# multiview-stitcher/multiview-stitcher

Hardware: AMD Instinct MI355X
Metric: Mvoxels/s register+fuse, 3D tile grid (higher is better)
Workload: dtype u16 in/out, f32 accumulate, f64 coordinates

## Files before the change

### multiview-stitcher_amd/csrc/mvs_context.hip

```cpp
#include "mvs_internal.h"
#include <vector>
#include <algorithm>

#include <algorithm>
#include <cstring>

static MvsContext g_ctx[MVS_MAX_DEVICES * MVS_MAX_LANES];

MvsContext* mvs_ctx(int device) {
    if (device < 0 || (device & 0xff) >= MVS_MAX_DEVICES || (device >> 8) >= MVS_MAX_LANES) return nullptr;
    return &g_ctx[mvs_ctx_index(device)];
}

int mvs_fail(MvsContext* c, int code, const char* fmt, ...) {
    char buf[1024];
    va_list ap;
    va_start(ap, fmt);
    vsnprintf(buf, sizeof(buf), fmt, ap);
    va_end(ap);
    if (c) { c->last_error = buf; c->last_code = code; }
    return code;
}

int mvs_check_ready(int device, MvsContext** out) {
// ... 126 lines not shown
    if (hipEventRecord(c->pinned_ev[k], c->stream) == hipSuccess) c->pinned_pending[k] = true;
    else hipStreamSynchronize(c->stream);
}

static size_t pool_round(uint64_t nbytes) {
    if (nbytes == 0) nbytes = 1;
    const size_t q = nbytes >= ((size_t)1 << 20) ? ((size_t)2 << 20) : 4096;
    return (nbytes + q - 1) / q * q;
}

static void pool_flush(MvsContext* c) {
    if (c->pool_free.empty()) return;
    hipStreamSynchronize(c->stream);
    for (auto& kv : c->pool_free) hipFree(kv.second);
    c->pool_free.clear();
    c->pool_cached_bytes = 0;
}

struct MvsBoolOption { const char* key; bool MvsContext::* field; };
static const MvsBoolOption kBoolOptions[] = {
    {"force_generic", &MvsContext::force_generic},
    {"no_regions", &MvsContext::no_regions},
    {"deconv_general", &MvsContext::deconv_general},
    {"dct_general", &MvsContext::dct_general},
    {"rows_v1", &MvsContext::rows_v1},
    {"cb_mask_count", &MvsContext::cb_mask_count},
    {"cb_mask_closed_form", &MvsContext::cb_mask_closed_form},
    {"fuse_mixed", &MvsContext::fuse_mixed},
    {"serial_classes", &MvsContext::serial_classes},
    {"reg_unfused", &MvsContext::reg_unfused},
    {"ssim_two_pass", &MvsContext::ssim_two_pass},
    {"ssim_f32", &MvsContext::ssim_f32},
    {"ssim_prune", &MvsContext::ssim_prune},
    {"materialize_shifts", &MvsContext::materialize_shifts},
    {"cb_exact", &MvsContext::cb_exact},
    {"cb_blend_generic", &MvsContext::cb_blend_generic},
    {"cb_nosplit", &MvsContext::cb_nosplit},
    {"cb_unpaired", &MvsContext::cb_unpaired},
    {"fft_no_pair", &MvsContext::fft_no_pair},
    {"fft_no_slab", &MvsContext::fft_no_slab},
    {"fft_no_line", &MvsContext::fft_no_line},
};
static int set_option(MvsContext* c, const char* key, int64_t value) {
    for (const MvsBoolOption& e : kBoolOptions)
        if (!strcmp(key, e.key)) {
            c->*e.field = value != 0;
            return MVS_OK;
        }
    if (!strcmp(key, "pool_cache_limit_mb")) {
        std::lock_guard<std::mutex> plock(c->pool_mu);
        c->pool_cache_limit = (size_t)std::max<int64_t>(value, 0) << 20;
        if (c->pool_cached_bytes > c->pool_cache_limit) pool_flush(c);
        return MVS_OK;
    }
    if (!strcmp(key, "cb_taps_f64")) {
        if (value < 0 || value > 3) return mvs_fail(c, MVS_ERR_INVALID_ARG, "mvs_set_option: cb_taps_f64 is 0, 1, 2 or 3");
        c->cb_taps = (int)value;
        return MVS_OK;
    }
    if (!strcmp(key, "fft_slab_axes")) {
        if (value < 0 || value > 7) return mvs_fail(c, MVS_ERR_INVALID_ARG, "mvs_set_option: fft_slab_axes is a mask of 3 bits");
        c->fft_slab_axes = (int)value;
        return MVS_OK;
    }
    if (!strcmp(key, "psf_batch")) {
        if (value < 0) return mvs_fail(c, MVS_ERR_INVALID_ARG, "mvs_set_option: psf_batch is 0 (automatic) or a number of beads");
        c->psf_batch = value;
        return MVS_OK;
    }
    if (!strcmp(key, "feather_slab_planes")) {
        if (value < 0) return mvs_fail(c, MVS_ERR_INVALID_ARG, "mvs_set_option: feather_slab_planes is 0 (automatic) or a number of planes");
        c->feather_slab_planes = value;
        return MVS_OK;
    }
    if (!strcmp(key, "ablate")) {
        c->ablate = (int)value;
        return MVS_OK;
    }
    return mvs_fail(c, MVS_ERR_INVALID_ARG, "mvs_set_option: unknown key '%s'", key);
}
struct MvsCounter { const char* key; double MvsContext::* real; long long MvsContext::* count; };
static const MvsCounter kCounters[] = {
    {"reg_alg_bytes", &MvsContext::reg_alg_bytes, nullptr},
    {"reg_alg_bytes_full", &MvsContext::reg_alg_bytes_full, nullptr},
    {"reg_pairs", nullptr, &MvsContext::reg_pairs},
    {"reg_candidates", nullptr, &MvsContext::reg_candidates},
    {"reg_rewalks", nullptr, &MvsContext::reg_rewalks},
    {"reg_pruned", nullptr, &MvsContext::reg_pruned},
    {"reg_cand_volumes", &MvsContext::reg_cand_volumes, nullptr},
    {"reg_slab_pairs", nullptr, &MvsContext::reg_slab_pairs},
    {"reg_rank_hist", nullptr, &MvsContext::reg_rank_hist},
    {"reg_rank_sort16", nullptr, &MvsContext::reg_rank_sort16},
    {"reg_rank_sort32", nullptr, &MvsContext::reg_rank_sort32},
    {"cb_mask_views", nullptr, &MvsContext::cb_mask_views},
    {"cb_mask_boxes", nullptr, &MvsContext::cb_mask_boxes},
    {"cb_line_launches", nullptr, &MvsContext::cb_line_launches},
    {"cb_overflows_redone", nullptr, &MvsContext::cb_overflows},
    {"cb_exact_chunks", nullptr, &MvsContext::cb_exact_chunks},
    {"cb_exact_large_chunks", nullptr, &MvsContext::cb_exact_large_chunks},
    {"cb_exact_paired_launches", nullptr, &MvsContext::cb_exact_paired_launches},
    {"cb_exact_lds_launches", nullptr, &MvsContext::cb_exact_lds_launches},
    {"cb_exact_tap_launches", nullptr, &MvsContext::cb_exact_tap_launches},
    {"fuse_rows_chunks", nullptr, &MvsContext::fuse_rows_chunks},
    {"fuse_region_chunks", nullptr, &MvsContext::fuse_region_chunks},
    {"fuse_column_chunks", nullptr, &MvsContext::fuse_column_chunks},
    {"fuse_generic_chunks", nullptr, &MvsContext::fuse_generic_chunks},
    {"fuse_weighted_chunks", nullptr, &MvsContext::fuse_weighted_chunks},
};

extern "C" {

const char* mvs_version(void) { return "mvs_hip 0.1 (gfx950)"; }

int mvs_device_count(void) {
    int n = 0;
    if (hipGetDeviceCount(&n) != hipSuccess) return 0;
    return n;
}

int mvs_init(int device) {
    MvsContext* c = mvs_ctx(device);
// ... 21 lines not shown
            hipDeviceProp_t prop;
            MVS_HIP_TRY(c, hipGetDeviceProperties(&prop, mvs_hip_device(device)));
            const int ncu = prop.multiProcessorCount;
            const bool xcd = !strncmp(ev, "xcd", 3);
            const int k = std::max(1, std::min(8, atoi(ev + (xcd ? 3 : 6))));
            std::vector<uint32_t> mask((size_t)(ncu + 31) / 32, 0u);
            for (int i = 0; i < ncu; ++i) {
                bool on;
                if (xcd) { const int x = i % 8, first = (lane * k) % 8; on = ((x - first + 8) % 8) < k; }
                else { const int slot = (i / 8) % 8, first = (lane * k) % 8; on = ((slot - first + 8) % 8) < k; }
                if (on) mask[(size_t)i / 32] |= 1u << (i % 32);
            }
            if (hipExtStreamCreateWithCUMask(&c->own_stream, (uint32_t)mask.size(), mask.data()) == hipSuccess) masked = true;
            else (void)hipGetLastError();
        }
        if (!masked) MVS_HIP_TRY(c, hipStreamCreateWithFlags(&c->own_stream, hipStreamNonBlocking));
    }
    MVS_HIP_TRY(c, hipEventCreate(&c->ev_start));
    MVS_HIP_TRY(c, hipEventCreate(&c->ev_stop));
    MVS_HIP_TRY(c, hipEventCreateWithFlags(&c->pinned_ev[0], hipEventDisableTiming));
    MVS_HIP_TRY(c, hipEventCreateWithFlags(&c->pinned_ev[1], hipEventDisableTiming));
    c->pinned_pending[0] = c->pinned_pending[1] = false;
    c->stream = c->own_stream;
    c->device = device;
    c->pool_cache_limit = ((device >> 8) ? (size_t)4 : (size_t)32) << 30;
    if (((device >> 8) & 0xff) == 0) {
        size_t f = 0, t = 0;
        if (hipMemGetInfo(&f, &t) == hipSuccess) c->pool_cache_limit = std::max(c->pool_cache_limit, t / 2);
        else (void)hipGetLastError();
    }
    {
        static const char* const env_switch[][2] = {{"MVS_SSIM_PRUNE", "ssim_prune"},   {"MVS_SSIM_F32", "ssim_f32"},
                                                    {"MVS_FUSE_MIXED", "fuse_mixed"},   {"MVS_FFT_SLAB_AXES", "fft_slab_axes"},
                                                    {"MVS_FFT_NO_SLAB", "fft_no_slab"}, {"MVS_FFT_NO_PAIR", "fft_no_pair"}};
        for (const auto& e : env_switch) {
            const char* ev = getenv(e[0]);
            if (ev && *ev) (void)set_option(c, e[1], atoi(ev));
        }
    }
    c->ready = true;
    c->last_error.clear();
    c->last_code = 0;
    return MVS_OK;
}

#ifdef MVS_PROFILING_ABLATIONS
extern "C++" bool mvs_dup_kernel(const char* tag) {
    static const std::string list = [] { const char* e = getenv("MVS_DUP_KERNELS"); return std::string(",") + (e ? e : "") + ","; }();
    return list.find(std::string(",") + tag + ",") != std::string::npos;
}
#endif

void mvs_shutdown(int device) {
    MvsContext* c = mvs_ctx(device);
    if (!c || !c->ready) return;
    std::lock_guard<std::recursive_mutex> lock(c->mu);
    hipSetDevice(mvs_hip_device(device));
    hipStreamSynchronize(c->stream);
    if (((device >> 8) & 0xff) == 0) mvs_transfer_shutdown(mvs_hip_device(device));
    {
        std::lock_guard<std::mutex> plock(c->pool_mu);
        for (auto& kv : c->pool_free) hipFree(kv.second);
        c->pool_free.clear();
        c->pool_cached_bytes = 0;
        c->pool_live.clear();
    }
    for (auto& s : c->dev) {
// ... 376 lines not shown
```

### multiview-stitcher_amd/csrc/mvs_internal.h

```cpp
#pragma once
#include <hip/hip_runtime.h>

#include <cstdarg>
#include <cstdint>
#include <cstdio>
#include <map>
#include <mutex>
#include <unordered_map>
#include <string>
#include <vector>

#include "mvs_hip.h"

#define MVS_MAX_DEVICES 16
#define MVS_MAX_LANES 16
static inline int mvs_hip_device(int id) { return id & 0xff; }
static inline int mvs_ctx_index(int id) { return ((id >> 8) & 0xff) * MVS_MAX_DEVICES + (id & 0xff); }

struct MvsScratch {
    void* ptr = nullptr;
    size_t cap = 0;
};

struct MvsContext {
    int device = -1;
    bool ready = false;
    hipStream_t own_stream = nullptr;
    hipStream_t stream = nullptr;
    hipEvent_t ev_start = nullptr, ev_stop = nullptr;
    bool timing_valid = false;
    int ablate = 0;
    bool force_generic = false;
    double reg_alg_bytes = 0.0;
    double reg_alg_bytes_full = 0.0;
    long long reg_pairs = 0, reg_candidates = 0, reg_pruned = 0;
    long long reg_slab_pairs = 0;
    long long reg_rank_hist = 0, reg_rank_sort16 = 0, reg_rank_sort32 = 0;
    double reg_cand_volumes = 0.0;
    hipStream_t aux_stream[4] = {nullptr, nullptr, nullptr, nullptr};
    hipEvent_t ev_fork = nullptr, ev_join[4] = {nullptr, nullptr, nullptr, nullptr};
    bool fuse_mixed = false;
    bool serial_classes = false;
    bool reg_unfused = false;
    bool ssim_f32 = true;
    long long reg_rewalks = 0;
    bool ssim_prune = true;
    bool fft_no_pair = false;
    bool ssim_two_pass = false;
    bool materialize_shifts = false;
    std::recursive_mutex mu;
    std::string last_error;
    MvsScratch dev[16];
    void* pinned = nullptr;
    size_t pinned_cap = 0;
    void* pinned2 = nullptr;
    size_t pinned2_cap = 0;
    hipEvent_t pinned_ev[2] = {nullptr, nullptr};
    hipEvent_t ticket_ev[32] = {};
    uint32_t ticket_next = 0;
    bool pinned_pending[2] = {false, false};
    int last_code = 0;
    void* mbox_host = nullptr;
    void* mbox_dev = nullptr;
    size_t mbox_cap = 0;
    uint64_t mbox_gen = 0;
    bool cb_mask_closed_form = false;
    bool cb_mask_count = false;
    long long cb_mask_views = 0, cb_mask_boxes = 0;
    bool cb_exact = false;
    bool cb_blend_generic = false;
    int cb_taps = 1;
    int* cb_flag_host = nullptr;
    int* cb_flag_dev = nullptr;
    long long cb_overflows = 0, cb_line_launches = 0;
    long long cb_exact_chunks = 0, cb_exact_large_chunks = 0, cb_exact_paired_launches = 0, cb_exact_lds_launches = 0, cb_exact_tap_launches = 0;
    bool cb_nosplit = false;
    bool cb_unpaired = false;
    int fft_slab_axes = 4;
// ... 130 lines not shown
```

### multiview-stitcher_amd/csrc/mvs_prune_search.h

```cpp
#pragma once

#include <algorithm>
#include <cmath>

#if defined(__HIPCC__)
#define MVS_WALK_HD __host__ __device__
#else
#define MVS_WALK_HD
#endif

constexpr int kSelRot = 7;

struct WalkItem { int tx, ty, zs, z0, z1, y0, x0; };

template <int WIN>
struct WalkGeom {
    static constexpr int TY = 16, TX = 56, H = WIN / 2, PAD = (WIN - 1) / 2;
    static constexpr int kMinSeg = 8;
    int nz, ny, nx, zseg, cz, cy, cx, nty, ntx, nzs, nitems;

    MVS_WALK_HD static constexpr int crop(int n) { return n - 2 * PAD; }
    MVS_WALK_HD static constexpr int lesser(int a, int b) { return a < b ? a : b; }
    MVS_WALK_HD static constexpr int tiles(int ny, int nx) { return ((crop(ny) + TY - 1) / TY) * ((crop(nx) + TX - 1) / TX); }
    MVS_WALK_HD WalkGeom(int nz_, int ny_, int nx_, int zseg_)
        : nz(nz_), ny(ny_), nx(nx_), zseg(zseg_), cz(crop(nz_)), cy(crop(ny_)), cx(crop(nx_)), nty((cy + TY - 1) / TY), ntx((cx + TX - 1) / TX),
          nzs((cz + zseg_ - 1) / zseg_), nitems(nty * ntx * nzs) {}
    MVS_WALK_HD WalkItem item(int i) const {
        WalkItem w;
        w.tx = i % ntx; w.ty = (i / ntx) % nty; w.zs = i / (ntx * nty);
        w.z0 = PAD + w.zs * zseg;
        w.z1 = lesser(w.z0 + zseg, nz - PAD);
        w.y0 = PAD + w.ty * TY; w.x0 = PAD + w.tx * TX;
        return w;
    }
    MVS_WALK_HD static int group_first(int grp, int K) { return grp * K; }
    MVS_WALK_HD static int rotated(int res, int grp, int K) { return (res + kSelRot * grp) % K; }
    MVS_WALK_HD static int item_of(int grp, int res, int K) { return group_first(grp, K) + rotated(res, grp, K); }
    MVS_WALK_HD static int residue_of(int item, int K) { return (((item % K) - kSelRot * (item / K)) % K + K) % K; }
    MVS_WALK_HD double voxels(int i) const {
        const WalkItem w = item(i);
        return (double)(w.z1 - w.z0) * (double)lesser(TY, cy - w.ty * TY) * (double)lesser(TX, cx - w.tx * TX);
    }
    static int zseg_for(int nz, int ny, int nx, int budget, int sharers = 1) {
        const int cz = crop(nz);
        const int nzs = std::max(1, std::min(budget / std::max(tiles(ny, nx) * sharers, 1), (cz + kMinSeg - 1) / kMinSeg));
        return (cz + nzs - 1) / nzs;
    }
};

constexpr int kPruneMaxCand = 16;
constexpr double kPruneMarginF32 = 1e-3;

template <int WIN>
inline void prune_residue_volumes(const WalkGeom<WIN>& g, int K, double vol_res[32]) {
    for (int r = 0; r < 32; ++r) vol_res[r] = 0.0;
    for (int item = 0; item < g.nitems; ++item) vol_res[WalkGeom<WIN>::residue_of(item, K)] += g.voxels(item);
}

class PruneSearch {
public:
    PruneSearch(int n, const bool* takes_part, int K, const double vol_res[32], double Ntot, double slack, double margin, double im1_min)
        : nb(n), K(K), kAll(K == 32 ? 0xffffffffu : 0xffffu), Ntot(Ntot), slack(slack), margin(margin), im1_min(im1_min) {
        for (int r = 0; r < 32; ++r) this->vol_res[r] = vol_res[r];
        for (int j = 0; j < kPruneMaxCand; ++j) {
            in[j] = j < n && takes_part[j];
            acc[j] = 0.0; amx[j] = -INFINITY; ahn[j] = 0; done[j] = 0; masks[j] = 0; dropped[j] = false; again[j] = false; ub[j] = 0.0; racc[j] = 0.0;
        }
    }

    bool next_round(unsigned int out[kPruneMaxCand]) {
        bool more = false;
        if (phase == kFirst) {
            for (int j = 0; j < nb; ++j) { masks[j] = in[j] ? 0x0001u : 0u; more = more || in[j]; }
        } else if (phase == kRounds && round < 34) {
            more = plan();
        }
        if (!more && phase != kFirst && phase != kOver) {
            more = phase == kRounds && select_rewalk();
            phase = more ? kRewalk : kOver;
        }
        for (int j = 0; j < kPruneMaxCand; ++j) out[j] = more ? masks[j] : 0u;
// ... 103 lines not shown
```

### multiview-stitcher_amd/csrc/mvs_score.hip

```cpp
#include "mvs_internal.h"
#include "mvs_fold_dev.h"
#include "mvs_prune_search.h"
#include "mvs_rank_plan.h"

#include <cstring>

#include <rocprim/rocprim.hpp>

#include <cmath>
#include <cstdlib>
#include <vector>

namespace {

constexpr int kStatBlocks = 1024;
constexpr int kMaxResident = 16;
static_assert(kMaxResident == kPruneMaxCand, "PruneSearch holds one batch");
constexpr int kChunk = 8;

inline int grid_for(long long n) { return mvs_rank_plan::score_grid(n); }

struct Shape3 { int nz, ny, nx; };

struct VoxStats { unsigned long long cnt; int bb[6]; };
// ... 210 lines not shown
                if (fabsf(v) == INFINITY) cnt += 1ull << 32;
                mnz = min(mnz, z); mny = min(mny, y); mnx = min(mnx, x);
                mxz = max(mxz, z); mxy = max(mxy, y); mxx = max(mxx, x);
            }
            if (++x == S.nx) { x = 0; if (++y == S.ny) { y = 0; ++z; } }
        }
    }
    block_reduce_voxstats(cnt, mnz, mny, mnx, mxz, mxy, mxx, partial + blockIdx.x);
}

__device__ __forceinline__ int reflect_index(int p, int len) {
    if (len == 1) return 0;
    const int period = 2 * len;
    p %= period;
    if (p < 0) p += period;
    if (p >= len) p = period - 1 - p;
    return p;
}

template <int WIN, int NOUT, typename ACC = double>
__device__ __forceinline__ void box_means(const float (&v)[NOUT + WIN - 1], float (&out)[NOUT]) {
    constexpr ACC inv = (ACC)(1.0 / (double)WIN);
    ACC d[NOUT + WIN - 1];
#pragma unroll
    for (int k = 0; k < NOUT + WIN - 1; ++k) d[k] = (ACC)v[k];
    ACC run = (ACC)0;
#pragma unroll
    for (int j = 0; j < WIN; ++j) run += d[j];
    out[0] = (float)(run * inv);
#pragma unroll
    for (int k = 1; k < NOUT; ++k) {
        run += d[k + WIN - 1] - d[k - 1];
        out[k] = (float)(run * inv);
    }
}

struct Five { const float* src[5]; float* dst[5]; };

struct ShiftArg { double tz, ty, tx; int skip_zero_taps; };
template <int WIN, bool SHIFTED, int QSET = 0>
__device__ __forceinline__ void ssim_first_pass_body(const float* __restrict__ im0, const float* __restrict__ im1t, Shape3 S,
                                                              int lz, int ly, int lx, Shape3 R, int axis, Five P,
                                                              float* __restrict__ pmax, int* __restrict__ phasnan, ShiftArg T) {
    constexpr int H = WIN / 2, NL = kChunk + 2 * H;
    const int len = axis == 0 ? R.nz : R.ny;
    const int nchunks = (len + kChunk - 1) / kChunk;
    const unsigned int other = axis == 0 ? (unsigned int)R.ny : (unsigned int)R.nz;
    const unsigned int items = (unsigned int)nchunks * other * (unsigned int)R.nx;
    const int src_stride = axis == 0 ? S.ny * S.nx : S.nx;
    const int dst_stride = axis == 0 ? R.ny * R.nx : R.nx;
    float mx = -INFINITY;
    int hn = 0;
    for (unsigned int w = blockIdx.x * blockDim.x + threadIdx.x; w < items; w += gridDim.x * blockDim.x) {
        const int x = (int)(w % (unsigned int)R.nx);
        const unsigned int t = w / (unsigned int)R.nx;
        int z, y, p0;
        if (axis == 0) { y = (int)(t % other); p0 = (int)(t / other) * kChunk; z = 0; }
        else { p0 = (int)(t % (unsigned int)nchunks) * kChunk; z = (int)(t / (unsigned int)nchunks); y = 0; }
        const int src_base = ((z + lz) * S.ny + (y + ly)) * S.nx + (x + lx);
        float va[NL], vb[NL];
        AxisTap TX = {0, 0, 0, 0.0}, TO = {0, 0, 0, 0.0};
        if (SHIFTED) {
            TX = axis_tap(x + lx, T.tx, S.nx);
            TO = axis == 0 ? axis_tap(y + ly, T.ty, S.ny) : axis_tap(z + lz, T.tz, S.nz);
        }
#pragma unroll
// ... 175 lines not shown
                        acc += (double)((A1 * A2) / (B1 * B2));
                    }
                }
            }
            __syncthreads();
        }
    }
    for (int off = 32; off > 0; off >>= 1) acc += __shfl_down(acc, off);
    __shared__ double sred[4];
    if ((threadIdx.x & 63) == 0) sred[threadIdx.x >> 6] = acc;
    __syncthreads();
    if (MODE != 1 && threadIdx.x == 0) partial[blockIdx.x] = sred[0] + sred[1] + sred[2] + sred[3];
}

template <int WIN, int MODE = 0>
__global__ __launch_bounds__(256) void ssim_yx_fused_kernel(Five P, Shape3 R, float cov_norm, float C1, float C2, double* __restrict__ partial) {
    ssim_yx_fused_body<WIN, MODE>(P, R, cov_norm, C1, C2, partial);
}

struct YxCand { const float* src1; const float* src3; const float* src4; };
struct YxBatch { YxCand c[kMaxResident]; };
template <int WIN>
__global__ __launch_bounds__(256) void ssim_yx_batch_kernel(YxBatch B, float* __restrict__ ux, float* __restrict__ uxx, Shape3 R,
                                                            float cov_norm, float C1, float C2, double* __restrict__ partial) {
    const YxCand& C = B.c[blockIdx.y];
    if (!C.src1) return;
    Five P;
    for (int a = 0; a < 5; ++a) { P.src[a] = nullptr; P.dst[a] = nullptr; }
    P.src[1] = C.src1; P.src[3] = C.src3; P.src[4] = C.src4;
    P.dst[0] = ux; P.dst[2] = uxx;
    ssim_yx_fused_body<WIN, 2>(P, R, cov_norm, C1, C2, partial + (size_t)blockIdx.y * kStatBlocks);
}

struct FusedCand { const float* src; int dz, dy, dx; unsigned int sel; };
struct FusedBatch { FusedCand c[kMaxResident]; };
#ifndef MVS_SSIM_WPE_LO
#define MVS_SSIM_WPE_LO 3
#define MVS_SSIM_WPE_HI 4
#endif
template <int WIN, bool F32>
__device__ __forceinline__ void ssim_fused_batch_body(const float* __restrict__ im0, Shape3 S, const FusedBatch& B,
                                                               const float* __restrict__ ux, const float* __restrict__ uxx, int zseg,
                                                               float cov_norm, float C1, float C2, float* __restrict__ pmax,
                                                               int* __restrict__ phasnan, double* __restrict__ psum, int selk) {
    typedef WalkGeom<WIN> G;
    constexpr int H = G::H, pad = G::PAD, TY = G::TY, TX = G::TX, LY = TY + 2 * H, LX = TX + 2 * H;
    constexpr int NO = 4, NI = NO + 2 * H;
    constexpr int NR = (LY + 3) / 4;
    typedef typename std::conditional<F32, float, double>::type run_t;
    constexpr run_t inv = (run_t)(1.0 / (double)WIN);
    static_assert(LX <= 64 && TY % NO == 0 && TX % NO == 0 && (TY * TX) / NO <= 256 && TY / NO == 4, "tile layout");
    __shared__ float sz_[3][LY][LX + 1];
    __shared__ float sy_[3][TY][LX + 1];
    const FusedCand C = B.c[blockIdx.y];
    const int nselres = __popc(C.sel);
    if (!C.src || nselres == 0) return;
    const int tid = threadIdx.x, col = tid & 63, wrow = tid >> 6;
    const int cz = S.nz - 2 * pad, cy = S.ny - 2 * pad, cx = S.nx - 2 * pad;
    float mx = -INFINITY;
    int hn = 0;
    unsigned long long nanmask = 0;
    double acc = 0.0;
    const long long vol_bytes = (long long)S.nz * S.ny * S.nx * 4;
    const __amdgpu_buffer_rsrc_t r0 = __builtin_amdgcn_make_buffer_rsrc((void*)im0, 0, (int)vol_bytes, 0x00020000);
    const __amdgpu_buffer_rsrc_t r1 = __builtin_amdgcn_make_buffer_rsrc((void*)C.src, 0, (int)vol_bytes, 0x00020000);
    if (cz > 0 && cy > 0 && cx > 0) {
        const G g(S.nz, S.ny, S.nx, zseg);
// ... 98 lines not shown
                        float f[3][NO];
#pragma unroll
                        for (int a = 0; a < 3; ++a) {
                            float v[NI];
#pragma unroll
                            for (int k = 0; k < NI; ++k) v[k] = sy_[a][row][ch * NO + k];
                            box_means<WIN, NO, run_t>(v, f[a]);
                        }
#pragma unroll
                        for (int k = 0; k < NO; ++k) {
                            if (x0 + ch * NO + k >= S.nx - pad) continue;
                            const float a = fa[k], axx = faxx[k], b = f[0][k];
                            const float vx = cov_norm * (axx - a * a);
                            const float vy = cov_norm * (f[1][k] - b * b);
                            const float vxy = cov_norm * (f[2][k] - a * b);
                            const float A1 = 2.f * a * b + C1, A2 = 2.f * vxy + C2;
                            const float B1 = a * a + b * b + C1, B2 = vx + vy + C2;
                            acc += (double)((A1 * A2) / (B1 * B2));
                        }
                    }
                }
            }
            __syncthreads();
        }
    }
    if (nanmask) hn = 1;
    const RegionStats r = mvs_fold::block_fold<4>(RegionStats{mx, hn, acc});
    if (tid == 0) {
        const size_t o = (size_t)blockIdx.y * kStatBlocks + blockIdx.x;
        pmax[o] = r.mx; phasnan[o] = r.hasnan; psum[o] = r.ssim_sum;
    }
}

#ifndef MVS_SSIM_F32_WPE_LO
#define MVS_SSIM_F32_WPE_LO 3
#define MVS_SSIM_F32_WPE_HI 4
#endif
template <int WIN, bool F32 = false>
__global__ __launch_bounds__(256) __attribute__((amdgpu_waves_per_eu(MVS_SSIM_WPE_LO, MVS_SSIM_WPE_HI)))
void ssim_fused_batch_kernel(const float* __restrict__ im0, Shape3 S, FusedBatch B, const float* __restrict__ ux, const float* __restrict__ uxx, int zseg,
                             float cov_norm, float C1, float C2, float* __restrict__ pmax, int* __restrict__ phasnan, double* __restrict__ psum, int selk) {
    ssim_fused_batch_body<WIN, false>(im0, S, B, ux, uxx, zseg, cov_norm, C1, C2, pmax, phasnan, psum, selk);
}
template <int WIN>
__global__ __launch_bounds__(256) __attribute__((amdgpu_waves_per_eu(MVS_SSIM_F32_WPE_LO, MVS_SSIM_F32_WPE_HI)))
void ssim_fused_batch_f32_kernel(const float* __restrict__ im0, Shape3 S, FusedBatch B, const float* __restrict__ ux, const float* __restrict__ uxx, int zseg,
                                 float cov_norm, float C1, float C2, float* __restrict__ pmax, int* __restrict__ phasnan, double* __restrict__ psum, int selk) {
    ssim_fused_batch_body<WIN, true>(im0, S, B, ux, uxx, zseg, cov_norm, C1, C2, pmax, phasnan, psum, selk);
}

template <int WIN>
__global__ __launch_bounds__(256) __attribute__((amdgpu_waves_per_eu(4, 8)))
void ssim_fixed_walk_kernel(const float* __restrict__ im0, Shape3 S, float* __restrict__ ux, float* __restrict__ uxx, int zseg) {
    typedef WalkGeom<WIN> G;
    constexpr int H = G::H, pad = G::PAD, TY = G::TY, TX = G::TX, LY = TY + 2 * H, LX = TX + 2 * H;
    constexpr int NO = 4, NI = NO + 2 * H;
    constexpr int NR = (LY + 3) / 4;
    constexpr double inv = 1.0 / (double)WIN;
    static_assert(LX <= 64 && TY % NO == 0 && TX % NO == 0 && (TY * TX) / NO <= 256 && TY / NO == 4, "tile layout");
    __shared__ float sz_[2][LY][LX + 1];
    __shared__ float sy_[2][TY][LX + 1];
    const int tid = threadIdx.x, col = tid & 63, wrow = tid >> 6;
    if (G::crop(S.nz) <= 0 || G::crop(S.ny) <= 0 || G::crop(S.nx) <= 0) return;
    const long long vol_bytes = (long long)S.nz * S.ny * S.nx * 4;
    const __amdgpu_buffer_rsrc_t r0 = __builtin_amdgcn_make_buffer_rsrc((void*)im0, 0, (int)vol_bytes, 0x00020000);
    const G g(S.nz, S.ny, S.nx, zseg);
    const int sy = S.nx, sz = S.ny * S.nx;
    for (int item = blockIdx.x; item < g.nitems; item += gridDim.x) {
        const WalkItem w = g.item(item);
        const int z0 = w.z0, z1 = w.z1, y0 = w.y0, x0 = w.x0;
        const int gx = min(x0 - H + col, S.nx - 1);
        int v0[NR];
#pragma unroll
        for (int k = 0; k < NR; ++k) {
            const int gy = min(y0 - H + min(wrow + 4 * k, LY - 1), S.ny - 1);
            v0[k] = (gy * sy + gx) * 4;
        }
        double s1[NR], s2[NR];
#pragma unroll
        for (int k = 0; k < NR; ++k) { s1[k] = 0.0; s2[k] = 0.0; }
        float an[NR], ao[NR];
// ... 686 lines not shown
                const bool half = half_shift(t, &H);
                bool fresh = false;
                const int q = half ? share_cls(sc, H, &fresh) : -1;
                if (q >= 0) {
                    b.cls_of[j] = q;
                    if (fresh)
                        shift_batch.c[n_shift_batch++] = ShiftCand{sc.cls[q].buf, 0.5 * H.hz, 0.5 * H.hy, 0.5 * H.hx, 1, HalfShift{0, 0, 0, H.hz, H.hy, H.hx}};
                    continue;
                }
                shift_batch.c[n_shift_batch++] = half ? ShiftCand{sc.im1t_buf[j], t[0], t[1], t[2], 1, H}
                                                      : ShiftCand{sc.im1t_buf[j], t[0], t[1], t[2], 0, HalfShift{0, 0, 0, 0, 0, 0}};
                sc.resident[b.ics[j]] = j;
                continue;
            }
        }
        launch_shift_copy(sc, b, j);
    }
    if (n_shift_batch)
        MVS_DUP("shift", hipLaunchKernelGGL(shift_batch_kernel, dim3(kStatBlocks, n_shift_batch), dim3(256), 0, c->stream, sc.im1, sc.im0, sc.S, shift_batch, sc.im1_all_finite));
    if (!sc.on_the_fly) {
        hipLaunchKernelGGL(finish_voxstats_kernel, dim3(b.nb), dim3(256), 0, c->stream, sc.vox_partial, sc.vox_out);
        MVS_HIP_TRY(c, hipStreamSynchronize(c->stream));
        for (int j = 0; j < b.nb; ++j) b.h_vs[j] = sc.h_vox[j];
    }
    return MVS_OK;
}

int ssim_window(const ScoreCall& sc, Shape3 R) {
    int min_shape = 0x7fffffff;
    for (int k = sc.k0; k < 3; ++k) min_shape = std::min(min_shape, (&R.nz)[k]);
    return std::min(7, min_shape - ((min_shape - 1) % 2));
}

void phase_b(ScoreCall& sc, ScoreBatch& b) {
    MvsContext* c = sc.c;
    const Shape3 S = sc.S;
    const int* bb0 = sc.h_im[0].bb;
    b.any_batched = false;
    b.cov_norm = 0.f;
    for (int j = 0; j < kMaxResident; ++j) {
        b.first.c[j] = FirstCand{nullptr, nullptr, nullptr, nullptr, ShiftArg{0.0, 0.0, 0.0, 0}, 0};
        b.yx.c[j] = YxCand{nullptr, nullptr, nullptr};
        b.fused.c[j] = FusedCand{nullptr, 0, 0, 0, 0xffffffffu};
        b.scored[j] = false;
        b.Rs[j] = {0, 0, 0};
    }
    for (int j = 0; j < b.nb; ++j) {
        const int ic = b.ics[j];
        const unsigned long long cnt = b.h_vs[j].cnt;
        const int* bb1 = b.h_vs[j].bb;
        sc.cnts[ic] = cnt;
        if (cnt == 0 || (double)cnt / (double)sc.valid1 < 0.1) {
            sc.code_out[ic] = 1;
            continue;
        }
        int lo[3], hi[3];
        for (int k = 0; k < 3; ++k) {
            if (sc.region_mode == 0) { lo[k] = std::min(bb0[k], bb1[k]); hi[k] = std::max(bb0[3 + k], bb1[3 + k]) + 1; }
            else { lo[k] = std::max(bb0[k], bb1[k]); hi[k] = std::min(bb0[3 + k], bb1[3 + k]) + 1; }
        }
        const Shape3 R = {std::max(hi[0] - lo[0], 0), std::max(hi[1] - lo[1], 0), std::max(hi[2] - lo[2], 0)};
        b.Rs[j] = R;
        if ((long long)R.nz * R.ny * R.nx <= 0) continue;
        const int win = std::max(ssim_window(sc, R), 3);
        double NP = 1.0;
        for (int k = 0; k < sc.ndim; ++k) NP *= (double)win;
        const float cov_norm = (float)(NP / (NP - 1.0));
        float* pm = sc.pmax + (size_t)j * kStatBlocks;
        int* ph = sc.phasnan + (size_t)j * kStatBlocks;
        double* ps = sc.psum + (size_t)j * kStatBlocks;
        const bool full = R.nz == S.nz && R.ny == S.ny && R.nx == S.nx;
        const bool joins = b.batched && win == 7 && full;
        if (b.cls_of[j] >= 0 && !joins) {
            launch_shift_copy(sc, b, j);
            b.cls_of[j] = -1;
        }
        const float* second = b.otf[j] ? sc.im1 : sc.im1t_buf[j];
        const ShiftArg* sa = b.otf[j] ? &b.shifts[j] : nullptr;
        if (joins) {
            float* d1 = sc.cand3[(size_t)3 * j], *d3 = sc.cand3[(size_t)3 * j + 1], *d4 = sc.cand3[(size_t)3 * j + 2];
            const ShiftArg& T = b.shifts[j];
            b.first.c[j] = FirstCand{second, d1, d3, d4, T, b.otf[j] ? 1 : 0};
            b.yx.c[j] = YxCand{d1, d3, d4};
            b.fused.c[j] = b.otf[j] ? FusedCand{sc.im1, (int)T.tz, (int)T.ty, (int)T.tx, 0xffffffffu}
                           : b.cls_of[j] >= 0 ? FusedCand{sc.cls[b.cls_of[j]].buf, (int)std::floor(T.tz), (int)std::floor(T.ty), (int)std::floor(T.tx), 0xffffffffu}
                                              : FusedCand{sc.im1t_buf[j], 0, 0, 0, 0xffffffffu};
            b.any_batched = true;
            b.cov_norm = cov_norm;
        }
        else if (win == 7) launch_ssim_passes<7>(c->stream, sc.im0, second, S, lo, R, sc.ndim, sc.setA, sc.setB, cov_norm, sc.C1, sc.C2, pm, ph, ps, sa, sc.shared_x && full);
        else if (win == 5) launch_ssim_passes<5>(c->stream, sc.im0, second, S, lo, R, sc.ndim, sc.setA, sc.setB, cov_norm, sc.C1, sc.C2, pm, ph, ps, sa);
        else launch_ssim_passes<3>(c->stream, sc.im0, second, S, lo, R, sc.ndim, sc.setA, sc.setB, cov_norm, sc.C1, sc.C2, pm, ph, ps, sa);
        b.scored[j] = true;
    }
}

void score_full(ScoreCall& sc, ScoreBatch& b, int n_in) {
    MvsContext* c = sc.c;
    const Shape3 S = sc.S;
    MVS_DUP("ssim_fused", hipLaunchKernelGGL(ssim_fused_batch_kernel<7>, dim3(kStatBlocks, b.nb), dim3(256), 0, c->stream, sc.im0, S, b.fused, sc.setB[2], sc.setB[3],
                       Walk7::zseg_for(S.nz, S.ny, S.nx, 1536, b.nb), b.cov_norm, sc.C1, sc.C2, sc.pmax, sc.phasnan, sc.psum, 32));
    c->reg_cand_volumes += (double)n_in;
}

void score_two_pass(ScoreCall& sc, ScoreBatch& b) {
    MvsContext* c = sc.c;
    hipLaunchKernelGGL(ssim_first_pass_batch_kernel<7>, dim3(kStatBlocks, b.nb), dim3(256), 0, c->stream, sc.im0, sc.S, b.first, sc.pmax, sc.phasnan);
    hipLaunchKernelGGL(ssim_yx_batch_kernel<7>, dim3(kStatBlocks, b.nb), dim3(256), 0, c->stream, b.yx, sc.setB[2], sc.setB[3], sc.S, b.cov_norm, sc.C1, sc.C2, sc.psum);
}

struct PruneEnv { int target_items, K; bool debug; };
const PruneEnv& prune_env() {
    static const PruneEnv env = [] {
        const char* items = getenv("MVS_SSIM_PRUNE_ITEMS");
        const char* classes = getenv("MVS_SSIM_PRUNE_CLASSES");
        return PruneEnv{(items && atoi(items) > 0) ? atoi(items) : 320, (classes && atoi(classes) == 16) ? 16 : 32, getenv("MVS_PRUNE_DEBUG") != nullptr};
    }();
    return env;
}

int run_round(ScoreCall& sc, const ScoreBatch& b, const Walk7& g, int K, const unsigned int* masks, bool f32) {
    MvsContext* c = sc.c;
    FusedBatch fb = b.fused;
    int maxsel = 0;
    for (int j = 0; j < b.nb; ++j) {
        fb.c[j].sel = masks[j];
        if (!masks[j]) { fb.c[j].src = nullptr; continue; }
        maxsel = std::max(maxsel, ((g.nitems + K - 1) / K) * __builtin_popcount(masks[j]));
    }
    const int gx = std::min(kStatBlocks, maxsel);
    if (f32)
        MVS_DUP("ssim_fused", hipLaunchKernelGGL(ssim_fused_batch_f32_kernel<7>, dim3(gx, b.nb), dim3(256), 0, c->stream, sc.im0, sc.S, fb, sc.setB[2], sc.setB[3], g.zseg,
                           b.cov_norm, sc.C1, sc.C2, sc.pmax, sc.phasnan, sc.psum, K));
    else
        MVS_DUP("ssim_fused", hipLaunchKernelGGL(ssim_fused_batch_kernel<7>, dim3(gx, b.nb), dim3(256), 0, c->stream, sc.im0, sc.S, fb, sc.setB[2], sc.setB[3], g.zseg,
                           b.cov_norm, sc.C1, sc.C2, sc.pmax, sc.phasnan, sc.psum, K));
    MVS_DUP("finish", hipLaunchKernelGGL(finish_region_kernel, dim3(b.nb), dim3(256), 0, c->stream, sc.pmax, sc.phasnan, sc.psum, sc.reg_out, gx));
    MVS_HIP_TRY(c, hipStreamSynchronize(c->stream));
    return MVS_OK;
}

int score_pruned(ScoreCall& sc, ScoreBatch& b, double slack) {
    MvsContext* c = sc.c;
    const Shape3 S = sc.S;
    const PruneEnv& env = prune_env();
    const Walk7 g(S.nz, S.ny, S.nx, Walk7::zseg_for(S.nz, S.ny, S.nx, env.target_items));
    double vol_res[32];
    prune_residue_volumes(g, env.K, vol_res);
    const double Ntot = (double)g.cz * (double)g.cy * (double)g.cx;
    bool in[kMaxResident];
    for (int j = 0; j < kMaxResident; ++j) in[j] = b.fused.c[j].src != nullptr;
    const bool walk_f32 = c->ssim_f32;
    PruneSearch search(b.nb, in, env.K, vol_res, Ntot, slack, walk_f32 ? kPruneMarginF32 : 0.0, sc.im1_min);
    unsigned int masks[kMaxResident];
    while (search.next_round(masks)) {
        if (search.rewalk())
            for (int j = 0; j < b.nb; ++j)
                if (masks[j]) { c->reg_rewalks += 1; c->reg_cand_volumes += 1.0; }
        const int rc = run_round(sc, b, g, env.K, masks, walk_f32 && !search.rewalk());
        if (rc) return rc;
        double sum[kMaxResident];
        float mx[kMaxResident];
        int hasnan[kMaxResident];
        for (int j = 0; j < b.nb; ++j) { sum[j] = sc.h_reg[j].ssim_sum; mx[j] = sc.h_reg[j].mx; hasnan[j] = sc.h_reg[j].hasnan; }
        search.take(sum, mx, hasnan);
// ... 327 lines not shown
```

Baseline: 102,800.

## Add packed-f32x2 fused SSIM kernel with interior fast path for candidate walks

Adds a new f32 fused SSIM body that handles pairs of rows as two-wide float vectors and shares the box-mean sums for mean and square terms. It uses buffer loads and a per-candidate valid box, so tiles lying fully inside it take a lean path with no bounds or NaN checks. The new path is on by default when the f32 SSIM mode is used. The aim is to cut ALU and bounds-check overhead in the dominant registration scoring kernel, at the cost of extra shared memory, more kernel complexity and a new correctness surface.

```diff
diff --git a/multiview-stitcher_amd/csrc/mvs_context.hip b/multiview-stitcher_amd/csrc/mvs_context.hip
--- a/multiview-stitcher_amd/csrc/mvs_context.hip
+++ b/multiview-stitcher_amd/csrc/mvs_context.hip
@@ -182,6 +182,7 @@
     {"ssim_two_pass", &MvsContext::ssim_two_pass},
     {"ssim_f32", &MvsContext::ssim_f32},
     {"ssim_prune", &MvsContext::ssim_prune},
+    {"ssim_pack", &MvsContext::ssim_pack},
     {"materialize_shifts", &MvsContext::materialize_shifts},
     {"cb_exact", &MvsContext::cb_exact},
     {"cb_blend_generic", &MvsContext::cb_blend_generic},
@@ -237,6 +238,8 @@
     {"reg_candidates", nullptr, &MvsContext::reg_candidates},
     {"reg_rewalks", nullptr, &MvsContext::reg_rewalks},
     {"reg_pruned", nullptr, &MvsContext::reg_pruned},
+    {"reg_walk_interior", nullptr, &MvsContext::reg_walk_interior},
+    {"reg_walk_border", nullptr, &MvsContext::reg_walk_border},
     {"reg_cand_volumes", &MvsContext::reg_cand_volumes, nullptr},
     {"reg_slab_pairs", nullptr, &MvsContext::reg_slab_pairs},
     {"reg_rank_hist", nullptr, &MvsContext::reg_rank_hist},
@@ -324,7 +327,8 @@
     {
         static const char* const env_switch[][2] = {{"MVS_SSIM_PRUNE", "ssim_prune"},   {"MVS_SSIM_F32", "ssim_f32"},
                                                     {"MVS_FUSE_MIXED", "fuse_mixed"},   {"MVS_FFT_SLAB_AXES", "fft_slab_axes"},
-                                                    {"MVS_FFT_NO_SLAB", "fft_no_slab"}, {"MVS_FFT_NO_PAIR", "fft_no_pair"}};
+                                                    {"MVS_FFT_NO_SLAB", "fft_no_slab"}, {"MVS_FFT_NO_PAIR", "fft_no_pair"},
+                                                    {"MVS_SSIM_PACK", "ssim_pack"}};
         for (const auto& e : env_switch) {
             const char* ev = getenv(e[0]);
             if (ev && *ev) (void)set_option(c, e[1], atoi(ev));
diff --git a/multiview-stitcher_amd/csrc/mvs_internal.h b/multiview-stitcher_amd/csrc/mvs_internal.h
--- a/multiview-stitcher_amd/csrc/mvs_internal.h
+++ b/multiview-stitcher_amd/csrc/mvs_internal.h
@@ -44,6 +44,8 @@
     bool reg_unfused = false;
     bool ssim_f32 = true;
     long long reg_rewalks = 0;
+    bool ssim_pack = true;
+    long long reg_walk_interior = 0, reg_walk_border = 0;
     bool ssim_prune = true;
     bool fft_no_pair = false;
     bool ssim_two_pass = false;
diff --git a/multiview-stitcher_amd/csrc/mvs_prune_search.h b/multiview-stitcher_amd/csrc/mvs_prune_search.h
--- a/multiview-stitcher_amd/csrc/mvs_prune_search.h
+++ b/multiview-stitcher_amd/csrc/mvs_prune_search.h
@@ -33,6 +33,10 @@
         w.y0 = PAD + w.ty * TY; w.x0 = PAD + w.tx * TX;
         return w;
     }
+    MVS_WALK_HD bool interior(const WalkItem& w, const int lo[3], const int hi[3]) const {
+        return w.z0 - H >= lo[0] && w.z1 + H - 1 <= hi[0] && w.y0 - H >= lo[1] && lesser(w.y0 + TY + H - 1, ny - 1) <= hi[1] &&
+               w.x0 - H >= lo[2] && lesser(w.x0 + TX + H - 1, nx - 1) <= hi[2];
+    }
     MVS_WALK_HD static int group_first(int grp, int K) { return grp * K; }
     MVS_WALK_HD static int rotated(int res, int grp, int K) { return (res + kSelRot * grp) % K; }
     MVS_WALK_HD static int item_of(int grp, int res, int K) { return group_first(grp, K) + rotated(res, grp, K); }
@@ -47,6 +51,13 @@
         return (cz + nzs - 1) / nzs;
     }
 };
+
+inline void walk_candidate_box(const int dims[3], const int slo[3], const int shi[3], const int d[3], int lo[3], int hi[3]) {
+    for (int k = 0; k < 3; ++k) {
+        lo[k] = std::max(std::max(slo[k], 0) - d[k], 0);
+        hi[k] = std::min(std::min(shi[k], dims[k] - 1) - d[k], dims[k] - 1);
+    }
+}
 
 constexpr int kPruneMaxCand = 16;
 constexpr double kPruneMarginF32 = 1e-3;
diff --git a/multiview-stitcher_amd/csrc/mvs_score.hip b/multiview-stitcher_amd/csrc/mvs_score.hip
--- a/multiview-stitcher_amd/csrc/mvs_score.hip
+++ b/multiview-stitcher_amd/csrc/mvs_score.hip
@@ -266,6 +266,47 @@
     for (int k = 1; k < NOUT; ++k) {
         run += d[k + WIN - 1] - d[k - 1];
         out[k] = (float)(run * inv);
+    }
+}
+
+typedef float f32x2 __attribute__((ext_vector_type(2)));
+
+template <int WIN, int NOUT>
+__device__ __forceinline__ void box_means_pair(const f32x2 (&d)[NOUT + WIN - 1], f32x2 (&out)[NOUT]) {
+    constexpr float inv = (float)(1.0 / (double)WIN);
+    f32x2 run = f32x2{0.f, 0.f};
+#pragma unroll
+    for (int j = 0; j < WIN; ++j) run += d[j];
+    out[0] = run * inv;
+#pragma unroll
+    for (int k = 1; k < NOUT; ++k) {
+        run += d[k + WIN - 1] - d[k - 1];
+        out[k] = run * inv;
+    }
+}
+
+template <int WIN, int NOUT>
+__device__ __forceinline__ void box_means_line(const float (&v)[NOUT + WIN - 1], float (&out)[NOUT]) {
+    static_assert(NOUT % 2 == 0, "outputs in pairs");
+    constexpr float inv = (float)(1.0 / (double)WIN);
+    float diff[NOUT + 1];
+    diff[0] = 0.f;
+#pragma unroll
+    for (int k = 1; k < NOUT; k += 2) {
+        const f32x2 dd = f32x2{v[k + WIN - 1], v[k + WIN < NOUT + WIN - 1 ? k + WIN : k + WIN - 1]} - f32x2{v[k - 1], v[k]};
+        diff[k] = dd.x; diff[k + 1] = dd.y;
+    }
+    float run = 0.f;
+#pragma unroll
+    for (int j = 0; j < WIN; ++j) run += v[j];
+    float r[NOUT];
+    r[0] = run;
+#pragma unroll
+    for (int k = 1; k < NOUT; ++k) { run += diff[k]; r[k] = run; }
+#pragma unroll
+    for (int k = 0; k < NOUT; k += 2) {
+        const f32x2 o = f32x2{r[k], r[k + 1]} * inv;
+        out[k] = o.x; out[k + 1] = o.y;
     }
 }
 
@@ -507,7 +548,7 @@
     ssim_yx_fused_body<WIN, 2>(P, R, cov_norm, C1, C2, partial + (size_t)blockIdx.y * kStatBlocks);
 }
 
-struct FusedCand { const float* src; int dz, dy, dx; unsigned int sel; };
+struct FusedCand { const float* src; int dz, dy, dx; unsigned int sel; int lo[3], hi[3]; };
 struct FusedBatch { FusedCand c[kMaxResident]; };
 #ifndef MVS_SSIM_WPE_LO
 #define MVS_SSIM_WPE_LO 3
@@ -672,6 +713,181 @@
     }
 }
 
+template <int WIN>
+__device__ __forceinline__ void ssim_fused_batch_packed_body(const float* __restrict__ im0, Shape3 S, const FusedBatch& B,
+                                                             const float* __restrict__ ux, const float* __restrict__ uxx, int zseg,
+                                                             float cov_norm, float C1, float C2, float* __restrict__ pmax,
+                                                             int* __restrict__ phasnan, double* __restrict__ psum, int selk) {
+    typedef WalkGeom<WIN> G;
+    constexpr int H = G::H, pad = G::PAD, TY = G::TY, TX = G::TX, LY = TY + 2 * H, LX = TX + 2 * H;
+    constexpr int NO = 4, NI = NO + 2 * H;
+    constexpr int NR = (LY + 3) / 4, NP = NR / 2;
+    constexpr float inv = (float)(1.0 / (double)WIN);
+    static_assert(LX <= 64 && TY % NO == 0 && TX % NO == 0 && (TY * TX) / NO <= 256 && TY / NO == 4 && NR % 2 == 0 && NO % 2 == 0, "tile layout");
+    __shared__ f32x2 sz13[LY][LX + 1];
+    __shared__ float sz4[LY][LX + 1];
+    __shared__ f32x2 sy13[TY][LX + 1];
+    __shared__ float sy4[TY][LX + 1];
+    const FusedCand C = B.c[blockIdx.y];
+    const int nselres = __popc(C.sel);
+    if (!C.src || nselres == 0) return;
+    const int tid = threadIdx.x, col = tid & 63, wrow = tid >> 6;
+    const int cz = S.nz - 2 * pad, cy = S.ny - 2 * pad, cx = S.nx - 2 * pad;
+    float mx = -INFINITY;
+    int hn = 0;
+    unsigned long long nanmask = 0;
+    double acc = 0.0;
+    const long long vol_bytes = (long long)S.nz * S.ny * S.nx * 4;
+    const __amdgpu_buffer_rsrc_t r0 = __builtin_amdgcn_make_buffer_rsrc((void*)im0, 0, (int)vol_bytes, 0x00020000);
+    const __amdgpu_buffer_rsrc_t r1 = __builtin_amdgcn_make_buffer_rsrc((void*)C.src, 0, (int)vol_bytes, 0x00020000);
+    const __amdgpu_buffer_rsrc_t ru = __builtin_amdgcn_make_buffer_rsrc((void*)ux, 0, (int)vol_bytes, 0x00020000);
+    const __amdgpu_buffer_rsrc_t ruu = __builtin_amdgcn_make_buffer_rsrc((void*)uxx, 0, (int)vol_bytes, 0x00020000);
+    if (cz > 0 && cy > 0 && cx > 0) {
+        const G g(S.nz, S.ny, S.nx, zseg);
+        const int nitems = g.nitems;
+        const int sy = S.nx, sz = S.ny * S.nx;
+        const int nsel = ((nitems + selk - 1) / selk) * nselres;
+        auto walk = [&](const WalkItem& w, auto lean_tag) __attribute__((always_inline)) {
+            constexpr bool LEAN = decltype(lean_tag)::value;
+            const int z0 = w.z0, z1 = w.z1, y0 = w.y0, x0 = w.x0;
+            const int gx = min(x0 - H + col, S.nx - 1);
+            const bool xin = LEAN || (unsigned)(gx + C.dx) < (unsigned)S.nx;
+            int v0[NR], v1[NR];
+            bool in1[NR], out1 = false;
+#pragma unroll
+            for (int k = 0; k < NR; ++k) {
+                const int prow = wrow + 4 * k;
+                const int gy = min(y0 - H + min(prow, LY - 1), S.ny - 1);
+                in1[k] = LEAN || (xin && (unsigned)(gy + C.dy) < (unsigned)S.ny);
+                v0[k] = (gy * sy + gx) * 4;
+                v1[k] = in1[k] ? ((gy + C.dy) * sy + gx + C.dx) * 4 : 0x7ffffff0;
+                out1 = out1 || (!in1[k] && prow < LY && col < LX);
+            }
+            if (out1) hn = 1;
+            f32x2 s1[NP], s3[NP], s4[NP];
+#pragma unroll
+            for (int j = 0; j < NP; ++j) { s1[j] = f32x2{0.f, 0.f}; s3[j] = f32x2{0.f, 0.f}; s4[j] = f32x2{0.f, 0.f}; }
+            f32x2 an[NP], bn[NP], ao[NP], bo[NP];
+            auto load_plane = [&](int p) __attribute__((always_inline)) {
+                const bool zin = LEAN || (unsigned)(p + C.dz) < (unsigned)S.nz;
+                const bool have_old = p - (z0 - H) >= WIN;
+                const bool zin_o = have_old && (LEAN || (unsigned)(p - WIN + C.dz) < (unsigned)S.nz);
+                if (!zin) hn = 1;
+                const int pn0 = p * sz * 4, pn1 = (p + C.dz) * sz * 4, po0 = (p - WIN) * sz * 4, po1 = (p - WIN + C.dz) * sz * 4;
+#pragma unroll
+                for (int k = 0; k < NR; ++k) {
+                    an[k / 2][k % 2] = __int_as_float(__builtin_amdgcn_raw_buffer_load_b32(r0, v0[k], pn0, 0));
+                    bn[k / 2][k % 2] = zin ? __int_as_float(__builtin_amdgcn_raw_buffer_load_b32(r1, v1[k], pn1, 0)) : 0.f;
+                    ao[k / 2][k % 2] = have_old ? __int_as_float(__builtin_amdgcn_raw_buffer_load_b32(r0, v0[k], po0, 0)) : 0.f;
+                    bo[k / 2][k % 2] = zin_o ? __int_as_float(__builtin_amdgcn_raw_buffer_load_b32(r1, v1[k], po1, 0)) : 0.f;
+                }
+            };
+            if (col < LX) load_plane(z0 - H);
+            const int xrow = tid / (TX / NO), xch = tid % (TX / NO);
+            const bool xact = tid < TY * (TX / NO) && y0 + xrow < S.ny - pad;
+            const int uoff = ((y0 + xrow) * S.nx + x0 + xch * NO) * 4;
+            for (int p = z0 - H; p < z1 + H; ++p) {
+                float fa[NO], faxx[NO];
+                if (xact && p >= z0 + H) {
+                    const int uplane = (p - H) * sz * 4;
+#pragma unroll
+                    for (int k = 0; k < NO; ++k) {
+                        fa[k] = __int_as_float(__builtin_amdgcn_raw_buffer_load_b32(ru, uoff + 4 * k, uplane, 0));
+                        faxx[k] = __int_as_float(__builtin_amdgcn_raw_buffer_load_b32(ruu, uoff + 4 * k, uplane, 0));
+                    }
+                }
+                if (col < LX) {
+#pragma unroll
+                    for (int j = 0; j < NP; ++j) {
+                        const int row0 = wrow + 8 * j, row1 = row0 + 4;
+                        const bool two = row1 < LY;
+                        const f32x2 a = an[j], a2 = ao[j];
+                        f32x2 b = bn[j], b2 = bo[j];
+                        if (LEAN) {
+                            mx = fmaxf(fmaxf(mx, b.x), b.y);
+                        } else {
+                            nanmask |= __ballot(b.x != b.x);
+                            mx = fmaxf(mx, in1[2 * j] ? b.x : -INFINITY);
+                            if (two) {
+                                nanmask |= __ballot(b.y != b.y);
+                                mx = fmaxf(mx, in1[2 * j + 1] ? b.y : -INFINITY);
+                            }
+                            b.x = (b.x != b.x) ? 0.f : b.x; b.y = (b.y != b.y) ? 0.f : b.y;
+                            b2.x = (b2.x != b2.x) ? 0.f : b2.x; b2.y = (b2.y != b2.y) ? 0.f : b2.y;
+                        }
+                        s1[j] += b - b2;
+                        s3[j] += b * b - b2 * b2;
+                        s4[j] += a * b - a2 * b2;
+                        if (p >= z0 + H) {
+                            const f32x2 m1 = s1[j] * inv, m3 = s3[j] * inv, m4 = s4[j] * inv;
+                            float* const q0 = reinterpret_cast<float*>(&sz13[row0][col]);
+                            q0[0] = m1.x; q0[1] = m3.x; sz4[row0][col] = m4.x;
+                            if (two) {
+                                float* const q1 = reinterpret_cast<float*>(&sz13[row1][col]);
+                                q1[0] = m1.y; q1[1] = m3.y; sz4[row1][col] = m4.y;
+                            }
+                        }
+                    }
+                    if (p + 1 < z1 + H) load_plane(p + 1);
+                }
+                if (p < z0 + H) continue;
+
+                __syncthreads();
+                if (col < LX) {
+                    f32x2 v13[NI], f13[NO];
+                    float v4[NI], f4[NO];
+#pragma unroll
+                    for (int k = 0; k < NI; ++k) { v13[k] = sz13[wrow * NO + k][col]; v4[k] = sz4[wrow * NO + k][col]; }
+                    box_means_pair<WIN, NO>(v13, f13);
+                    box_means_line<WIN, NO>(v4, f4);
+#pragma unroll
+                    for (int k = 0; k < NO; ++k) { sy13[wrow * NO + k][col] = f13[k]; sy4[wrow * NO + k][col] = f4[k]; }
+                }
+                __syncthreads();
+                if (xact) {
+                    f32x2 v13[NI], f13[NO];
+                    float v4[NI], f[3][NO];
+#pragma unroll
+                    for (int k = 0; k < NI; ++k) { v13[k] = sy13[xrow][xch * NO + k]; v4[k] = sy4[xrow][xch * NO + k]; }
+                    box_means_pair<WIN, NO>(v13, f13);
+                    box_means_line<WIN, NO>(v4, f[2]);
+#pragma unroll
+                    for (int k = 0; k < NO; ++k) { f[0][k] = f13[k].x; f[1][k] = f13[k].y; }
+#pragma unroll
+                    for (int k = 0; k < NO; k += 2) {
+                        const f32x2 a = f32x2{fa[k], fa[k + 1]}, axx = f32x2{faxx[k], faxx[k + 1]}, b = f32x2{f[0][k], f[0][k + 1]};
+                        const f32x2 vx = cov_norm * (axx - a * a);
+                        const f32x2 vy = cov_norm * (f32x2{f[1][k], f[1][k + 1]} - b * b);
+                        const f32x2 vxy = cov_norm * (f32x2{f[2][k], f[2][k + 1]} - a * b);
+                        const f32x2 A1 = 2.f * a * b + C1, A2 = 2.f * vxy + C2;
+                        const f32x2 B1 = a * a + b * b + C1, B2 = vx + vy + C2;
+                        const f32x2 num = A1 * A2, den = B1 * B2;
+                        if (x0 + xch * NO + k < S.nx - pad) acc += (double)(num.x / den.x);
+                        if (x0 + xch * NO + k + 1 < S.nx - pad) acc += (double)(num.y / den.y);
+                    }
+                }
+            }
+            __syncthreads();
+        };
+        for (int si = blockIdx.x; si < nsel; si += gridDim.x) {
+            unsigned int rest = C.sel;
+            for (int k = si % nselres; k > 0; --k) rest &= rest - 1;
+            const int grp = si / nselres;
+            const int item = G::group_first(grp, selk) + G::rotated(__ffs(rest) - 1, grp, selk);
+            if (item >= nitems) continue;
+            const WalkItem w = g.item(item);
+            if (g.interior(w, C.lo, C.hi)) walk(w, std::true_type());
+            else walk(w, std::false_type());
+        }
+    }
+    if (nanmask) hn = 1;
+    const RegionStats r = mvs_fold::block_fold<4>(RegionStats{mx, hn, acc});
+    if (tid == 0) {
+        const size_t o = (size_t)blockIdx.y * kStatBlocks + blockIdx.x;
+        pmax[o] = r.mx; phasnan[o] = r.hasnan; psum[o] = r.ssim_sum;
+    }
+}
+
 #ifndef MVS_SSIM_F32_WPE_LO
 #define MVS_SSIM_F32_WPE_LO 3
 #define MVS_SSIM_F32_WPE_HI 4
@@ -682,11 +898,12 @@
                              float cov_norm, float C1, float C2, float* __restrict__ pmax, int* __restrict__ phasnan, double* __restrict__ psum, int selk) {
     ssim_fused_batch_body<WIN, false>(im0, S, B, ux, uxx, zseg, cov_norm, C1, C2, pmax, phasnan, psum, selk);
 }
-template <int WIN>
+template <int WIN, bool PACK = false>
 __global__ __launch_bounds__(256) __attribute__((amdgpu_waves_per_eu(MVS_SSIM_F32_WPE_LO, MVS_SSIM_F32_WPE_HI)))
 void ssim_fused_batch_f32_kernel(const float* __restrict__ im0, Shape3 S, FusedBatch B, const float* __restrict__ ux, const float* __restrict__ uxx, int zseg,
                                  float cov_norm, float C1, float C2, float* __restrict__ pmax, int* __restrict__ phasnan, double* __restrict__ psum, int selk) {
-    ssim_fused_batch_body<WIN, true>(im0, S, B, ux, uxx, zseg, cov_norm, C1, C2, pmax, phasnan, psum, selk);
+    if constexpr (PACK) ssim_fused_batch_packed_body<WIN>(im0, S, B, ux, uxx, zseg, cov_norm, C1, C2, pmax, phasnan, psum, selk);
+    else ssim_fused_batch_body<WIN, true>(im0, S, B, ux, uxx, zseg, cov_norm, C1, C2, pmax, phasnan, psum, selk);
 }
 
 template <int WIN>
@@ -1439,6 +1656,23 @@
     return std::min(7, min_shape - ((min_shape - 1) % 2));
 }
 
+void set_candidate_box(const ScoreCall& sc, ScoreBatch& b, int j) {
+    FusedCand& F = b.fused.c[j];
+    const Shape3 S = sc.S;
+    const int dims[3] = {S.nz, S.ny, S.nx}, d[3] = {F.dz, F.dy, F.dx};
+    int slo[3] = {0, 0, 0}, shi[3] = {S.nz - 1, S.ny - 1, S.nx - 1};
+    if (!b.otf[j]) {
+        VoxStats vs = b.h_vs[j];
+        if (b.cls_of[j] >= 0) {
+            const ShiftArg& T = b.shifts[j];
+            const double frac[3] = {T.tz - std::floor(T.tz), T.ty - std::floor(T.ty), T.tx - std::floor(T.tx)};
+            vs = valid_box(S, frac);
+        }
+        for (int k = 0; k < 3; ++k) { slo[k] = vs.bb[k]; shi[k] = vs.bb[3 + k]; }
+    }
+    walk_candidate_box(dims, slo, shi, d, F.lo, F.hi);
+}
+
 void phase_b(ScoreCall& sc, ScoreBatch& b) {
     MvsContext* c = sc.c;
     const Shape3 S = sc.S;
@@ -1492,6 +1726,7 @@
             b.fused.c[j] = b.otf[j] ? FusedCand{sc.im1, (int)T.tz, (int)T.ty, (int)T.tx, 0xffffffffu}
                            : b.cls_of[j] >= 0 ? FusedCand{sc.cls[b.cls_of[j]].buf, (int)std::floor(T.tz), (int)std::floor(T.ty), (int)std::floor(T.tx), 0xffffffffu}
                                               : FusedCand{sc.im1t_buf[j], 0, 0, 0, 0xffffffffu};
+            set_candidate_box(sc, b, j);
             b.any_batched = true;
             b.cov_norm = cov_norm;
         }
@@ -1535,9 +1770,17 @@
         if (!masks[j]) { fb.c[j].src = nullptr; continue; }
         maxsel = std::max(maxsel, ((g.nitems + K - 1) / K) * __builtin_popcount(masks[j]));
     }
+    if (sc.so->state_out && f32)
+        for (int j = 0; j < b.nb; ++j)
+            for (int item = 0; masks[j] && item < g.nitems; ++item)
+                if ((masks[j] >> Walk7::residue_of(item, K)) & 1u)
+                    (g.interior(g.item(item), fb.c[j].lo, fb.c[j].hi) ? c->reg_walk_interior : c->reg_walk_border) += 1;
     const int gx = std::min(kStatBlocks, maxsel);
-    if (f32)
-        MVS_DUP("ssim_fused", hipLaunchKernelGGL(ssim_fused_batch_f32_kernel<7>, dim3(gx, b.nb), dim3(256), 0, c->stream, sc.im0, sc.S, fb, sc.setB[2], sc.setB[3], g.zseg,
+    if (f32 && c->ssim_pack)
+        MVS_DUP("ssim_fused", hipLaunchKernelGGL((ssim_fused_batch_f32_kernel<7, true>), dim3(gx, b.nb), dim3(256), 0, c->stream, sc.im0, sc.S, fb, sc.setB[2], sc.setB[3], g.zseg,
+                           b.cov_norm, sc.C1, sc.C2, sc.pmax, sc.phasnan, sc.psum, K));
+    else if (f32)
+        MVS_DUP("ssim_fused", hipLaunchKernelGGL((ssim_fused_batch_f32_kernel<7, false>), dim3(gx, b.nb), dim3(256), 0, c->stream, sc.im0, sc.S, fb, sc.setB[2], sc.setB[3], g.zseg,
                            b.cov_norm, sc.C1, sc.C2, sc.pmax, sc.phasnan, sc.psum, K));
     else
         MVS_DUP("ssim_fused", hipLaunchKernelGGL(ssim_fused_batch_kernel<7>, dim3(gx, b.nb), dim3(256), 0, c->stream, sc.im0, sc.S, fb, sc.setB[2], sc.setB[3], g.zseg,
```

Result: faster. 104,200 (median of 6 runs) (+1.3%).
